# dayne-2stacks/Fingerprint-Matching-Code

Measured on AMD Instinct MI355X. Metric: graph-match pairs/sec @ n=256 kpts, batch=1024, 1 & 8 GPU, higher is better.
Workload: dtype bf16

## Files before the change

### fingerprint-matching-code_amd/_lib.py

```python
import ctypes
import os

_HERE = os.path.dirname(os.path.abspath(__file__))
LIB_PATH = os.environ.get("FPM_LIB_PATH") or os.path.join(_HERE, "libfpm_hip.so")

P = ctypes.c_void_p
I = ctypes.c_int
L = ctypes.c_long
F = ctypes.c_float

SIGNATURES = {
    "fpm_last_error": (ctypes.c_char_p, []),
    "fpm_version": (I, []),
    "fpm_device_sync": (I, []),
    "fpm_sinkhorn_log_fwd": (I, [P, L, L, L, P, L, L, L, P, P, I, I, I, I, F, I, P]),
    "fpm_sinkhorn_ws_bytes": (L, [I, I, I]),
    "fpm_sinkhorn_log_fwd_ws": (I, [P, L, L, L, P, L, L, L, P, P, I, I, I, I, F, I, P, L, P]),
    "fpm_soft_topk_fwd": (I, [P, L, L, P, P, P, I, I, I, I, F, P, L, L, P, P, L, L, P]),
    "fpm_topk_select": (I, [P, L, L, P, L, P, I, I, I, P, L, L, P, L, L, P]),
    "fpm_greedy_perm": (I, [P, L, I, P, I, I, I, P, L, L, P]),
    "fpm_gemm": (I, [I, P, L, L, P, P, L, L, I, I, I, I, I, P, P, P, L, L, P, P, P]),
    "fpm_cast_bf16": (I, [P, P, L, P]),
    "fpm_global_weights": (I, [P, L, P, L, I, I, I, P, L, P]),
    "fpm_coef_tanh": (I, [P, L, P, P, I, I, I, P, L, P]),
# ... 44 lines not shown
    "fpm_match_cls_train_bwd": (I, [P, P, I, I, I] + [P] * 21 + [P]),
    "fpm_gemm_norm_max": (I, [P, L, P, L, I, I, I, P, P, L, P, P, ctypes.c_float, I, P, P]),
    "fpm_gemm_norm_out": (I, [P, L, P, L, I, I, I, P, P, P, ctypes.c_float, I, P, L, P, L, P]),
    "fpm_affinity_ws_floats": (L, [I, I, I]),
    "fpm_perm_loss_fwd": (I, [P, L, L, P, L, L, P, P, I, I, I, P, P, P, P]),
    "fpm_perm_loss_bwd": (I, [P, L, L, P, L, L, P, P, I, I, I, P, P, P, P]),
    "fpm_affinity_fwd": (I, [P, L, P, L, P, I, P, P, I, I, I, I, P, P, I, P, L, P, L, P]),
    "fpm_gemm_x3out": (I, [P, L, P, L, I, I, I, I, P, P, P, ctypes.c_float, I, P, L, P, L, I, P]),
    "fpm_lsa_batch_host": (I, [P, L, L, P, P, I, I, P, I]),
    "fpm_lsa_submit": (L, [P, L, L, P, P, I, I, P, I]),
    "fpm_lsa_wait": (I, [L, I, ctypes.POINTER(ctypes.c_double)]),
    "fpm_lsa_batch_device": (I, [P, L, L, P, P, I, I, I, P, P, P]),
    "fpm_csr_dot_csc_to_dense": (I, [I, P, P, P, P, P, P, L, L, L, P, P]),
    "fpm_dense_dot_csc_to_dense": (I, [I, P, P, P, P, L, L, L, L, P, P]),
    "fpm_csr_dot_diag_to_csr": (I, [I, P, P, P, P, L, L, L, P, P]),
    "fpm_bilinear_diag": (I, [I, P, P, P, P, L, P, P, P, L, L, P, P]),
    "fpm_csr_dot_csc_to_csr_host": (L, [I, P, P, P, P, P, P, L, L, L, P, L, P, P]),
    "fpm_csr_dot_diag_to_csr_host": (I, [I, P, P, P, P, L, L, L, P]),
    "fpm_bilinear_diag_host": (I, [I, P, P, P, P, L, P, P, P, L, L, P]),
    "fpm_gconv_ws_floats": (L, [I, I, I]),
    "fpm_gconv_fwd": (I, [P, P, I, I, I, I, P, P, I, P, P, P]),
    "fpm_graph_words": (I, [I]),
    "fpm_graph_build": (I, [P, P, I, I, I, ctypes.c_double, P, P, P, P, P]),
    "fpm_graph_edges": (I, [P, P, P, P, I, I, ctypes.c_double, P, P, P, P, P, P, I, P]),
    "fpm_kron_pattern": (I, [P, P, L, P, P, L, I, I, I, I, P, P, P]),
    "fpm_feature_align_ws_floats": (L, [P, P]),
    "fpm_feature_align_fwd": (I, [P, P, P, P, P, P, P, P, I, F, F, P, P, L, P, P]),
    "fpm_feature_align_bwd": (I, [P, P, P, P, P, P, P, P, I, F, F, P, P, L, P, P, P, P, P, P]),
    "fpm_sinkhorn_bwd_ws_floats": (L, [I, I, I, I]),
    "fpm_sinkhorn_log_bwd": (I, [P, L, L, L, P, L, L, L, P, P, P, I, I, I, I, F, I, P, L, P]),
    "fpm_soft_topk_bwd_ws_floats": (L, [I, I, I]),
    "fpm_soft_topk_bwd": (I, [P, L, L, P, P, P, P, I, I, I, F, P, L, L, P, P, L, P, P]),
    "fpm_spline_plan_rows": (I, [P, L, L, ctypes.POINTER(P), ctypes.POINTER(P)]),
    "fpm_spline_conv_bwd_data": (I, [I, P, L, L, I, P, P, P, I, P, P, P, P, P, P, I, P]),
    "fpm_gather_transpose": (I, [I, P, L, P, L, I, P, L, P]),
    "fpm_spline_weight_pack": (I, [P, P, I, I, I, I, I, P, P]),
    "fpm_spline_conv_bwd_data_scatter": (I, [I, P, P, P, L, L, I, P, P, P, I, P, P, P, P, P, P, I, P]),
    "fpm_kron_agg": (I, [P, I, I, I, I, P, P, P, P, P, P, P, P, I, P, P]),
    "fpm_kron_gnn_layer_bwd_point": (I, [P, I, I, I, I, P, P, P, P, P, P, P]),
    "fpm_kron_gnn_layer_fwd_f64": (I, [P, I, I, I, I, I, P, P, P, P, P, P, P, P, P, P]),
    "fpm_sinkhorn_log_fwd_f64": (I, [P, I, L, L, L, P, L, L, L, P, L, L, L, P, P, I, I, I, I, ctypes.c_double, I, P]),
    "fpm_node_classifier_f64": (I, [P, I, I, I, P, P, P, P, P]),
    "fpm_crossset_attn_row_f64": (I, [P, L, L, I, I, I, P, P, I, P, P, P, P, P, P]),
    "fpm_gemm_f64": (I, [P, I, P, I, P, P, I, I, I, I, I, P]),
    "fpm_instnorm_f64": (I, [P, P, I, I, I, P, P, P, P, ctypes.c_double, P, P, P]),
    "fpm_afau_head_f64": (I, [P, P, P, I, I, P, P, P, P, P, P, P, P, P, P]),
    "fpm_soft_topk_fwd_f64": (I, [P, L, L, P, P, P, I, I, I, I, ctypes.c_double, P, L, P, L, L, P, P, L, L, P]),
    "fpm_profile_enable": (I, [I]),
    "fpm_profile_enabled": (I, []),
    "fpm_profile_read": (I, [ctypes.POINTER(ctypes.c_double), ctypes.POINTER(ctypes.c_double),
                             ctypes.POINTER(I)]),
}

for _op, _probe in (("score", [P, I]), ("pairs", [P, P, P, I])):
    for _kernel, _ws in (("", []), ("_wide", [P, L]), ("_stream", [P, L])):
        for _rows in ("", "_rows16"):
            SIGNATURES["fpm_coarse_%s%s%s" % (_op, _kernel, _rows)] = (
                I, [P, P, P, I, I] + _probe + [P, I, F, P] + _ws + [P])

_lib = None


class FpmError(RuntimeError):
    pass


# ... 24 lines not shown
```

### fingerprint-matching-code_amd/csrc/gemm.hip

```cpp
#include "gemm_phase.h"
#include <cstdlib>
#include <cstring>

namespace fpm {
int& gemm_bn256_min();
}
int& gemm_store_sc1_flag();

extern "C" int fpm_gemm(int dtype, const void* A, long lda, long sA, const int* a_rows, const void* B, long ldb,
                        long sB, int M, int N, int K, int batch, int epi, const float* bias, float* Cf, void* Ct,
                        long ldc, long sC, const int* n1, const int* n2, void* stream) {
    using namespace fpm;
    FPM_CHECK_ARG(dtype == 0 || dtype == 1, "gemm: dtype must be 0 (f32) or 1 (bf16)");
    FPM_CHECK_ARG(M >= 0 && N > 0 && K > 0 && batch >= 0, "gemm: bad sizes M=%d N=%d K=%d", M, N, K);
    FPM_CHECK_ARG(K % (dtype ? 8 : 4) == 0, "gemm: K=%d must be a multiple of %d", K, dtype ? 8 : 4);
    FPM_CHECK_ARG(lda % (dtype ? 8 : 4) == 0 && ldb % (dtype ? 8 : 4) == 0, "gemm: lda/ldb must keep rows 16-B aligned");
    FPM_CHECK_ARG((epi != EPI_AFFINITY && epi != EPI_HALF_AFFINITY) || (n1 && n2),
                  "gemm: affinity epilogues need n1/n2");
    FPM_CHECK_ARG(epi >= EPI_STORE && epi <= EPI_HALF_AFFINITY, "gemm: bad epilogue %d", epi);
    if (M == 0 || batch == 0) return 0;
    GemmParams p = {};
    p.A = A; p.lda = lda; p.sA = sA; p.a_rows = a_rows;
    p.B = B; p.ldb = ldb; p.sB = sB; p.sB_seg = 0;
    p.row_scale = nullptr;
// ... 24 lines not shown
            else if (f32) FPM_BIG(256, EPI_STORE, true);
            else {
                const int S = phase ? gemm_walk_strip(p) : 0;
                p.store_sc1 = gemm_store_sc1_flag();
                if (S != 0) gemm_walk_launch(p, S, batch, st);
                else FPM_BIG(256, EPI_STORE, false);
            }
        } else {
            if (epi == EPI_RELU) { if (f32) FPM_BIG(128, EPI_RELU, true); else FPM_BIG(128, EPI_RELU, false); }
            else { if (f32) FPM_BIG(128, EPI_STORE, true); else FPM_BIG(128, EPI_STORE, false); }
        }
#undef FPM_BIG
        return check_launch("fpm_gemm");
    }
    p.remap_mtiles = (M + GBM - 1) / GBM;
    dim3 grid(remap_grid(N, p.remap_mtiles), 1, batch);
    if (dtype == 0) hipLaunchKernelGGL((gemm_kernel<float, false>), grid, dim3(GTHREADS), 0, st, p);
    else hipLaunchKernelGGL((gemm_kernel<bf16_t, false>), grid, dim3(GTHREADS), 0, st, p);
    return check_launch("fpm_gemm");
}

namespace fpm {
int& gemm_phase_flag() {
    static int on = [] {
        const char* e = getenv("FPM_GEMM_PHASE");
        return e ? atoi(e) : 1;
    }();
    return on;
}

int& gemm_walk_flag() {
    static int v = [] {
        const char* e = getenv("FPM_GEMM_WALK");
        return e ? atoi(e) : GW_AUTO;
    }();
    return v;
}

int gemm_cu_count() {
    static int cus = [] {
        int dev = 0, n = 0;
        if (hipGetDevice(&dev) != hipSuccess ||
            hipDeviceGetAttribute(&n, hipDeviceAttributeMultiprocessorCount, dev) != hipSuccess || n <= 0)
            n = 256;
        return n;
    }();
    return cus;
}

int& gemm_bn256_min() {
    static int v = [] {
        const char* e = getenv("FPM_GEMM_BN256_MIN");
        return e ? atoi(e) : 512;
    }();
    return v;
}
}

extern "C" int fpm_gemm_norm_max(const void* A, long lda, const void* B, long ldb, int M, int N, int K,
                                 const float* bias, const float* res, long ldres, const float* nw, const float* nb,
                                 float eps, int P, float* gmax, void* stream) {
    using namespace fpm;
    FPM_CHECK_ARG(P == G2_BM || 2 * P == G2_BM, "gemm_norm_max: P=%d must be %d or %d (one or two pairs per tile)", P,
                  G2_BM, G2_BM / 2);
    FPM_CHECK_ARG(M >= 0 && M % P == 0 && N > 0 && K > 0 && K % G2_BK == 0, "gemm_norm_max: bad sizes M=%d N=%d K=%d",
                  M, N, K);
    FPM_CHECK_ARG(lda % 8 == 0 && ldb % 8 == 0 && ldres >= N, "gemm_norm_max: bad strides");
// ... 126 lines not shown
    else if (key && !strcmp(key, "combine_npb")) f = &combine_npb_flag();
    else if (key && !strcmp(key, "sinkhorn_bwd_reg")) f = &sinkhorn_bwd_reg_flag();
    else if (key && !strcmp(key, "sinkhorn_fast")) f = &sinkhorn_fast_flag();
    else if (key && !strcmp(key, "sinkhorn_lform")) f = &sinkhorn_lform_flag();
    else if (key && !strcmp(key, "topk_fast")) f = &soft_topk_fast_flag();
    else if (key && !strcmp(key, "afau_attn_v")) f = &afau_attn_v_flag();
    else if (key && !strcmp(key, "gnn_store_sc1")) f = &gnn_store_sc1_flag();
    else if (key && !strcmp(key, "combine_store_sc1")) f = &combine_store_sc1_flag();
    else if (key && !strcmp(key, "gemm_store_sc1")) f = &gemm_store_sc1_flag();
    else if (key && !strcmp(key, "combine_lds_kb")) f = &combine_lds_kb_flag();
    else if (key && !strcmp(key, "gnn_mlp_off")) f = &gnn_mlp_off_flag();
    else if (key && !strcmp(key, "outer_sum_vec")) f = &outer_sum_vec_flag();
    else if (key && !strcmp(key, "gnn_sweeps")) f = &gnn_sweeps_flag();
    else if (key && !strcmp(key, "scatter_f32_rows")) f = &scatter_f32_rows_flag();
    else if (key && !strcmp(key, "scatter_batch")) f = &scatter_batch_flag();
    else if (key && !strcmp(key, "afau_head_split")) f = &afau_head_split_flag();
    if (!f) {
        fpm::set_error("fpm_set_tuning: unknown key '%s'", key ? key : "(null)");
        return -1;
    }
    if (f == &gnn_mlp_off_flag() && value != 0) {
        const char* e = getenv("FPM_TIMING_PROBES");
        if (!e || strcmp(e, "1") != 0) {
            fpm::set_error("fpm_set_tuning: '%s' is a timing probe with wrong results; set FPM_TIMING_PROBES=1 "
                           "to allow it", key);
            return -1;
        }
    }
    const int prev = *f;
    *f = value;
    return prev;
}

namespace {
__global__ void cast_bf16_kernel(const float* __restrict__ x, bf16_t* __restrict__ y, long n) {
    long i = (long)blockIdx.x * blockDim.x + threadIdx.x;
    long stride = (long)gridDim.x * blockDim.x;
    for (; i < n; i += stride) y[i] = fpm::f2bf(x[i]);
}

__global__ __launch_bounds__(256) void cast_bf16_v8_kernel(const float4* __restrict__ x, uint4* __restrict__ y, long n8) {
    const long i = (long)blockIdx.x * blockDim.x + threadIdx.x;
    if (i >= n8) return;
    const float4 a = x[2 * i], b = x[2 * i + 1];
    uint4 o;
    o.x = (uint32_t)fpm::f2bf(a.x) | ((uint32_t)fpm::f2bf(a.y) << 16);
    o.y = (uint32_t)fpm::f2bf(a.z) | ((uint32_t)fpm::f2bf(a.w) << 16);
    o.z = (uint32_t)fpm::f2bf(b.x) | ((uint32_t)fpm::f2bf(b.y) << 16);
    o.w = (uint32_t)fpm::f2bf(b.z) | ((uint32_t)fpm::f2bf(b.w) << 16);
    y[i] = o;
}
}

extern "C" int fpm_cast_bf16(const float* x, void* y, long n, void* stream) {
    if (n <= 0) return 0;
    if (n % 8 == 0 && ((uintptr_t)x & 15) == 0 && ((uintptr_t)y & 15) == 0) {
        const long n8 = n / 8;
        hipLaunchKernelGGL(cast_bf16_v8_kernel, dim3((unsigned)((n8 + 255) / 256)), dim3(256), 0, (hipStream_t)stream,
                           (const float4*)x, (uint4*)y, n8);
        return fpm::check_launch("fpm_cast_bf16");
    }
    long blocks = (n + 255) / 256;
    if (blocks > 65536) blocks = 65536;
    hipLaunchKernelGGL(cast_bf16_kernel, dim3(blocks), dim3(256), 0, (hipStream_t)stream, x, (bf16_t*)y, n);
    return fpm::check_launch("fpm_cast_bf16");
}
// ... 122 lines not shown
```

### fingerprint-matching-code_amd/csrc/gemm_core.h

```cpp
#pragma once
#include "fpm_common.h"

namespace fpm {

enum GemmEpi : int {
    EPI_STORE = 0,
    EPI_RELU = 1,
    EPI_TANH = 2,
    EPI_AFFINITY = 3,
    EPI_HALF_AFFINITY = 4,
    EPI_NORM_MAX = 5,
    EPI_NORM_OUT = 6,
};

struct GemmParams {
    const void* A;
    long lda, sA;
    const int* a_rows;
    const void* B;
    long ldb, sB, sB_seg;
    const float* row_scale;
    int M, N, K, nseg;
    const int* tile_info;
    const int* group_off;
    int epi;
    const float* bias;
    float* Cf;
    void* Ct;
    long ldc, sC;
    const int* n1;
    const int* n2;
    int remap_mtiles;
    const float* res;
    const float* nw;
    const float* nb;
    float eps;
    float* gmax;
    long ldt;
    int split;
    int norm_p;
    int store_sc1;
    int remap_cm;
    int walk;
    const int* tile_count;
    int walk_cus;
};

constexpr int REMAP_MIN = 32;
inline unsigned remap_grid(int N, int mtiles) {
    long nt = (N + 127) / 128, chunk = 4 * nt;
    long t = nt * mtiles;
    if (mtiles < REMAP_MIN) return (unsigned)t;
    return (unsigned)((t + 8 * chunk - 1) / (8 * chunk) * (8 * chunk));
}
__device__ __forceinline__ int remap_tile(int nt, int mtiles, int cm = 4) {
    if (mtiles < REMAP_MIN) return blockIdx.x;
    const int chunk = cm * nt;
    const int i = blockIdx.x >> 3;
    return ((i / chunk) * 8 + (blockIdx.x & 7)) * chunk + (i % chunk);
}

typedef __bf16 bf16x8_t __attribute__((ext_vector_type(8)));
typedef float f32x4_t __attribute__((ext_vector_type(4)));

template <typename T> struct TileCfg;
template <> struct TileCfg<float> {
    static constexpr int BK = 32;
    static constexpr int EPC = 4;
};
template <> struct TileCfg<bf16_t> {
    static constexpr int BK = 64;
    static constexpr int EPC = 8;
};

constexpr int GBM = 128, GBN = 128, GTHREADS = 256;
constexpr int LDS_ROW_BYTES = 144;
constexpr int LDS_TILE_BYTES = GBM * LDS_ROW_BYTES;

// ... 197 lines not shown
```

### fingerprint-matching-code_amd/csrc/gemm_phase.h

```cpp
#pragma once
#include <type_traits>
#include "gemm_big.h"

namespace fpm {

constexpr int GP_HALF = 128 * 128;
constexpr int GP_SMEM = g2_max(8 * GP_HALF, G2_BM * (2 * 256 + 16));
constexpr int GP_MIN_KTILES = 2;

#define FPM_VMCNT(N) asm volatile("s_waitcnt vmcnt(" #N ")" ::: "memory")

#ifdef GP_PROBE
__device__ unsigned long long* gp_probe_buf;
#define GP_STAMP(k)                                                                                   \
    do {                                                                                              \
        const unsigned long long t_ = __builtin_amdgcn_s_memtime();                                   \
        if (threadIdx.x == 0 && gp_probe_buf)                                                         \
            gp_probe_buf[((long)blockIdx.z * gridDim.x + blockIdx.x) * 8 + (k)] = t_;                   \
    } while (0)
#else
#define GP_STAMP(k)
#endif

#ifndef GP_STAGGER
// ... 271 lines not shown
                            *(float*)(smem + r * ROW + c * 4) =
                                g2_epi<EPI, HB>(p.bias, acc[h][g][fm][fn][j], row0 + h * 128 + r, n, n1b, n2b);
                        }
                    }
        };
#pragma unroll
        for (int h = 0; h < 2; ++h) {
            if (p.bias) image(h, std::true_type{});
            else image(h, std::false_type{});
            __syncthreads();
#pragma unroll 4
            for (int it = 0; it < 128 * CH / G2_THREADS; ++it) {
                const int idx = it * G2_THREADS + tid;
                const int r = idx / CH, ch = idx % CH;
                const int gr = row0 + h * 128 + r;
                if (gr < row_end && n0 + ch * 4 < p.N) {
                    uint4 v = *(const uint4*)(smem + r * ROW + ch * 16);
                    *(uint4*)(Cf + (long)gr * p.ldc + n0 + ch * 4) = v;
                }
            }
            __syncthreads();
        }
    }
}

constexpr int GW_SMEM = 8 * GP_HALF;
constexpr int GW_MAX_S = 2;

__host__ __device__ inline int gemm_walk_rule(int tiles, int wgs, int cus) {
    const long r1 = ((long)tiles * wgs + cus - 1) / cus, r2 = ((long)((tiles + 1) / 2) * wgs + cus - 1) / cus;
    return 2 * r2 * 7 <= r1 * 8 ? 2 : 1;
}

#ifdef GP_PROBE
#define GW_STAMP(k) do { if (ti == 0) GP_STAMP(k); } while (0)
#else
#define GW_STAMP(k)
#endif

template <bool SC1>
__global__ __launch_bounds__(G2_THREADS, 1) void gemm_walk_kernel(GemmParams p) {
    constexpr int BN = 256;
    __shared__ __attribute__((aligned(16))) unsigned char smem[GW_SMEM];
    const int tid = threadIdx.x, lane = tid & 63, wave = tid >> 6;
    const int wr = wave >> 2, wc = wave & 3;
    const int batch = blockIdx.z;

    const int nt = p.N / BN;
    int mtiles = p.remap_mtiles;
    if (p.tile_count) mtiles = *p.tile_count < mtiles ? *p.tile_count : mtiles;
    const int S = p.walk > 0 ? p.walk : gemm_walk_rule(mtiles, nt * (int)gridDim.z, p.walk_cus);
    const int strips = (mtiles + S - 1) / S;
    const int i = blockIdx.x >> 3;
    const int strip = (i / nt) * 8 + (blockIdx.x & 7), ntile = i % nt;
    if (strip >= strips) return;
    int t_row0[GW_MAX_S], t_rend[GW_MAX_S], t_grp[GW_MAX_S];
    unsigned ok = 0;
#pragma unroll
    for (int j = 0; j < GW_MAX_S; ++j) {
        const int mt = strip * S + j;
        t_row0[j] = 0; t_rend[j] = 0; t_grp[j] = 0;
        if (j < S && mt < mtiles) {
            if (p.tile_info) {
                const int g = p.tile_info[2 * mt];
                if (g >= 0) {
                    t_grp[j] = g;
                    t_row0[j] = p.tile_info[2 * mt + 1];
                    t_rend[j] = p.group_off[g + 1];
                    ok |= 1u << j;
                }
            } else {
                t_row0[j] = mt * G2_BM;
                t_rend[j] = p.M;
                ok |= 1u << j;
            }
        }
    }
    if (!ok) return;
    constexpr int m_end = GW_MAX_S;
    auto next_valid = [&](int j) __attribute__((always_inline)) {
        const unsigned r = j < GW_MAX_S ? ok >> j : 0u;
        return r ? j + __builtin_ctz(r) : GW_MAX_S;
    };
    auto pick = [&](const int (&t)[GW_MAX_S], int j) __attribute__((always_inline)) {
        return j == 0 ? t[0] : t[1];
    };
    int m = next_valid(0);

    const int n0 = ntile * BN;
    const bf16_t* A = (const bf16_t*)p.A + (long)batch * p.sA;
    const unsigned char* Bb = (const unsigned char*)((const bf16_t*)p.B + (long)batch * p.sB);
    bf16_t* Ct = (bf16_t*)p.Ct + (long)batch * p.sC;

// ... 203 lines not shown
    for (;;) {
        const bool has_next = mn < m_end;
        GW_STAMP(0);
        if (GP_STAGGER && wr == 1) __builtin_amdgcn_s_barrier();
        int k1 = G2_BK;
        for (int t = 0; t < T - 2; ++t, ++u, k1 += G2_BK) ktile(u, k1, 6, 6, 6, 6, CUR, CUR);
        ktile(u, k1, 6, 6, 6, has_next ? 6 : 4, CUR, has_next ? NEXT : NONE);
        GW_STAMP(1);
        ktile(u + 1, 0, has_next ? 6 : 2, has_next ? 6 : 0, -1, -1, has_next ? NEXT : NONE, NONE);
        ++u;
        if (GP_STAGGER && wr == 0) __builtin_amdgcn_s_barrier();
        GW_STAMP(2);
        if (p.bias) epilogue(u & 1, std::true_type{});
        else epilogue(u & 1, std::false_type{});
        GW_STAMP(3);
        if (!has_next) break;
        m = mn; mn = m_end;
        row0 = row0n; row_end = row_endn; bg = bgn;
#pragma unroll
        for (int h = 0; h < 2; ++h)
#pragma unroll
            for (int i = 0; i < 2; ++i) ar[h][i] = arn[h][i];
        issue(0, u & 1, ar, bg, G2_BK);
        issue(2, u & 1, ar, bg, G2_BK);
        FPM_VMCNT(4);
        zero_acc();
        __builtin_amdgcn_s_barrier();
        GW_STAMP(4);
        ++u;
#ifdef GP_PROBE
        ++ti;
#endif
    }
}

#undef FPM_VMCNT

int& gemm_phase_flag();
inline bool use_gemm_phase(int K) { return gemm_phase_flag() != 0 && K / G2_BK >= GP_MIN_KTILES; }

constexpr int GW_AUTO = 8;
int& gemm_walk_flag();
int gemm_cu_count();
inline int gemm_walk_strip(const GemmParams& p) {
    const int f = gemm_walk_flag();
    if (f <= 1 || !use_gemm_phase(p.K) || p.N % 256 != 0 || !p.Ct || p.Cf || p.epi != EPI_STORE) return 0;
    if ((long)p.N * p.ldb * 2 >= (1L << 31) || (long)G2_BM * p.ldc * 2 >= (1L << 31) || p.lda >= (1L << 31)) return 0;
    return f < GW_AUTO ? 2 : GW_AUTO;
}
inline void gemm_walk_launch(GemmParams p, int S, int batch, hipStream_t st) {
    const long nt = p.N / 256;
    p.walk_cus = gemm_cu_count();
    p.walk = S == 2 || p.remap_mtiles * nt * batch >= 8L * gemm_cu_count() ? 2 : 0;
    const int strips = p.walk ? (p.remap_mtiles + 1) / 2 : p.remap_mtiles;
    const dim3 grid((unsigned)((strips + 7) / 8 * 8 * nt), 1, batch);
    if (p.store_sc1) hipLaunchKernelGGL((gemm_walk_kernel<true>), grid, dim3(G2_THREADS), 0, st, p);
    else hipLaunchKernelGGL((gemm_walk_kernel<false>), grid, dim3(G2_THREADS), 0, st, p);
}

}
```

### fingerprint-matching-code_amd/csrc/spline.hip

```cpp
#include "gemm_phase.h"

#include <vector>

namespace {

struct ProfRec {
    hipEvent_t a, b;
    int slot;
};
bool g_prof_on = false;
std::vector<ProfRec> g_prof;
int* g_prof_rows = nullptr;
constexpr int PROF_MAX = 4096;

constexpr int NCELL = 26;

struct PlanLayout {
    long mask, indeg, dslot, basis_e, grp_e, blk_cnt, cell_off, rowid, arows, tile_info, tile_info2, dst_ptr, csr_e,
        nbr_local, rows4, basis4, total;
    long nblk, max_rows, max_tiles, max_tiles2;
};

__host__ __device__ inline long al(long x) { return (x + 255) & ~255L; }

// ... 1372 lines not shown
extern "C" int fpm_profile_enabled(void) { return g_prof_on ? 1 : 0; }

extern "C" int fpm_profile_read(double* ms_total, double* flops_total, int* count) {
    double ms = 0.0, fl = 0.0;
    for (auto& r : g_prof) {
        float t = 0.f;
        if (hipEventSynchronize(r.b) != hipSuccess || hipEventElapsedTime(&t, r.a, r.b) != hipSuccess) {
            fpm::set_error("fpm_profile_read: event query failed");
            return 2;
        }
        int rows = 0;
        if (hipMemcpy(&rows, g_prof_rows + r.slot, sizeof(int), hipMemcpyDeviceToHost) != hipSuccess) {
            fpm::set_error("fpm_profile_read: row count read failed");
            return 2;
        }
        ms += t;
        fl += 2.0 * rows * 768.0 * 768.0;
        (void)hipEventDestroy(r.a);
        (void)hipEventDestroy(r.b);
    }
    if (count) *count = (int)g_prof.size();
    g_prof.clear();
    if (ms_total) *ms_total = ms;
    if (flops_total) *flops_total = fl;
    return 0;
}

extern "C" int fpm_cast_bf16(const float* x, void* out, long n, void* stream);

extern "C" int fpm_spline_plan_rows(void* ws, long E, long num_nodes, int** arows, int** cell_off) {
    PlanLayout L = plan_layout(E, num_nodes);
    *arows = (int*)((char*)ws + L.arows);
    *cell_off = (int*)((char*)ws + L.cell_off);
    return 0;
}

extern "C" int fpm_spline_plan_edges(void* ws, long E, long num_nodes, int** csr_e, int** rows4, float** basis4) {
    PlanLayout L = plan_layout(E, num_nodes);
    *csr_e = (int*)((char*)ws + L.csr_e);
    *rows4 = (int*)((char*)ws + L.rows4);
    *basis4 = (float*)((char*)ws + L.basis4);
    return 0;
}

extern "C" int fpm_spline_conv_bwd_data_scatter(int dtype, const void* plan_ws, const void* rplan_ws,
                                                const int* argmax, long E, long num_nodes, int nmax,
                                                const int* nvalid, const void* Wb, const void* y_ws, int mode,
                                                const float* gout, const float* hout, float* dY, void* dY_op,
                                                float* dXrows, float* dX, int accumulate, void* stream);

extern "C" int fpm_spline_conv_bwd_data(int dtype, const void* plan_ws, long E, long num_nodes, int nmax,
                                        const int* nvalid, const void* Wb, const void* y_ws, int mode,
                                        const float* gout, const float* hout, float* dY, void* dY_op,
                                        float* dXrows, float* dX, int accumulate, void* stream) {
    return fpm_spline_conv_bwd_data_scatter(dtype, plan_ws, nullptr, nullptr, E, num_nodes, nmax, nvalid, Wb, y_ws,
                                            mode, gout, hout, dY, dY_op, dXrows, dX, accumulate, stream);
}

int& scatter_f32_rows_flag() {
    static int v = [] {
        const char* e = getenv("FPM_SCATTER_F32_ROWS");
        return e ? atoi(e) : 0;
    }();
    return v;
}

// ... 126 lines not shown
```

### fingerprint-matching-code_amd/ops.py

```python
import ctypes

import torch

from . import _lib

F32, BF16 = 0, 1
EPI_STORE, EPI_RELU, EPI_TANH, EPI_AFFINITY, EPI_HALF_AFFINITY = 0, 1, 2, 3, 4
EPI_NORM_OUT = 6


def _p(t):
    return ctypes.c_void_p(0 if t is None else t.data_ptr())


def _stream(t=None):
    dev = t.device if t is not None else torch.device("cuda")
    return ctypes.c_void_p(torch.cuda.current_stream(dev).cuda_stream)


def _dev(*ts):
    for t in ts:
        if t is not None and not t.is_cuda:
            raise _lib.FpmError("fpm op called with a CPU tensor: the HIP path has no CPU fallback")

# ... 1089 lines not shown
              dp.stride(1), dp.stride(2), _p(ds), _p(n1), _p(n2), B, n1max, n2max, int(iters), float(tau),
              int(bool(dummy_row)), _p(ws), ws.numel(), _stream(s))
    return ds


def soft_topk_bwd(ss, n1, n2, k, steps, tau, dds):
    _dev(ss, n1, n2, k, steps, dds)
    B, n1max, n2max = ss.shape
    if ss.stride(2) != 1 or dds.stride(2) != 1 or tuple(dds.shape) != (B, n1max, n2max):
        raise _lib.FpmError("soft_topk_bwd: (B, n1max, n2max) views with unit column stride expected")
    lib = _lib.load()
    ws = torch.empty(max(int(lib.fpm_soft_topk_bwd_ws_floats(B, n1max, n2max)), 1), device=ss.device,
                     dtype=torch.float32)
    status = torch.zeros(B, device=ss.device, dtype=torch.int32)
    dss = torch.empty(B, n1max, n2max, device=ss.device, dtype=torch.float32)
    _lib.call("fpm_soft_topk_bwd", _p(ss), ss.stride(0), ss.stride(1), _p(n1), _p(n2), _p(k), _p(steps), B, n1max,
              n2max, float(tau), _p(dds), dds.stride(0), dds.stride(1), _p(dss), _p(ws), ws.numel(), _p(status),
              _stream(ss))
    if int(status.sum()):
        raise _lib.FpmError("soft_topk_bwd: forward ran more steps than the backward replay holds")
    return dss


def spline_plan_rows(plan, E, num_nodes):
    a, c = ctypes.c_void_p(), ctypes.c_void_p()
    _lib.call("fpm_spline_plan_rows", _p(plan), E, num_nodes, ctypes.byref(a), ctypes.byref(c))
    base = plan.data_ptr()
    oa, oc = a.value - base, c.value - base
    arows = plan[oa:].view(torch.int32)
    cell_off = plan[oc:oc + 4 * 27].view(torch.int32)
    return arows, cell_off


def spline_plan_edges(plan, E, num_nodes):
    a, r, b = ctypes.c_void_p(), ctypes.c_void_p(), ctypes.c_void_p()
    _lib.call("fpm_spline_plan_edges", _p(plan), E, num_nodes, ctypes.byref(a), ctypes.byref(r), ctypes.byref(b))
    base = plan.data_ptr()
    oa, orr, ob = a.value - base, r.value - base, b.value - base
    csr_e = plan[oa:oa + 4 * E].view(torch.int32)
    rows4 = plan[orr:orr + 16 * E].view(torch.int32).view(E, 4)
    basis4 = plan[ob:ob + 16 * E].view(torch.float32).view(E, 4)
    return csr_e, rows4, basis4


def spline_conv_bwd_data(x_op, plan, E, num_nodes, nmax, nvalid, Wb, y_ws, mode, gout, hout, dY, dY_op, dXrows, dX,
                         accumulate=False, rplan=None, argmax=None):
    _dev(plan, nvalid, Wb, y_ws, gout, dY, dXrows, dX)
    code = _code(x_op)
    if _code(Wb) != code or tuple(Wb.shape) != (26, 768, 768):
        raise _lib.FpmError("spline_conv_bwd: Wb must be (26, 768, 768) in the operand dtype")
    if mode == 0 and hout is None:
        raise _lib.FpmError("spline_conv_bwd: mode 0 needs the layer output")
    if (rplan is None) != (argmax is None):
        raise _lib.FpmError("spline_conv_bwd: rplan and argmax go together")
    _lib.call("fpm_spline_conv_bwd_data_scatter", code, _p(plan), _p(rplan), _p(argmax), E, num_nodes, nmax,
              _p(nvalid), _p(Wb), _p(y_ws), int(mode), _p(gout), _p(hout), _p(dY), _p(dY_op), _p(dXrows), _p(dX),
              int(bool(accumulate)), _stream(gout))


def kron_agg(X, C, B, n1max, n2max, tcsr1, tcsr2, q1, q2, n1, n2, adjoint, out, accumulate=False):
    _dev(X, n1, n2, out)
    _lib.call("fpm_kron_agg", _p(X), int(C), int(B), int(n1max), int(n2max), ctypes.c_void_p(tcsr1[0]),
              ctypes.c_void_p(tcsr1[1]), ctypes.c_void_p(tcsr2[0]), ctypes.c_void_p(tcsr2[1]), ctypes.c_void_p(q1),
              ctypes.c_void_p(q2), _p(n1), _p(n2), int(bool(adjoint)) | (2 if accumulate else 0), _p(out), _stream(X))
    return out

# ... 104 lines not shown
```

### include/fpm.h

```cpp
#ifndef FPM_H_
#define FPM_H_

#ifdef __cplusplus
extern "C" {
#endif

const char* fpm_last_error(void);
int fpm_version(void);
int fpm_device_sync(void);

int fpm_sinkhorn_log_fwd(const float* s, long s_sb, long s_si, long s_sj, float* out, long o_sb, long o_si,
                         long o_sj, const int* n1, const int* n2, int B, int n1max, int n2max, int iters,
                         float tau, int dummy_row, void* stream);
long fpm_sinkhorn_ws_bytes(int B, int n1max, int n2max);
int fpm_sinkhorn_log_fwd_ws(const float* s, long s_sb, long s_si, long s_sj, float* out, long o_sb, long o_si,
                            long o_sj, const int* n1, const int* n2, int B, int n1max, int n2max, int iters,
                            float tau, int dummy_row, void* ws, long ws_bytes, void* stream);

int fpm_soft_topk_fwd(const float* ss, long s_sb, long s_ld, const int* n1, const int* n2, const float* k, int B,
                      int n1max, int n2max, int iters, float tau, float* out, long o_sb, long o_ld, int* steps_out,
                      float* out2, long o2_sb, long o2_ld, void* stream);

int fpm_topk_select(const float* ds, long d_sb, long d_ld, const int* assign, long a_sb, const float* k, int B,
                    int n1max, int n2max, float* perm, long p_sb, long p_ld, float* lsa_out, long l_sb, long l_ld,
// ... 226 lines not shown
                     float* score, void* stream);
int fpm_coarse_pairs_wide(const float* y, const long* row_off, const int* idx, int G, int B, const float* yq,
                          const long* qrow_off, const int* qidx, int Q, const float* coef, int iters, float tau,
                          float* score, void* ws, long ws_bytes, void* stream);
int fpm_coarse_pairs_stream(const float* y, const long* row_off, const int* idx, int G, int B, const float* yq,
                            const long* qrow_off, const int* qidx, int Q, const float* coef, int iters, float tau,
                            float* score, void* ws, long ws_bytes, void* stream);
int fpm_coarse_pairs_rows16(const void* y16, const long* row_off, const int* idx, int G, int B, const float* yq,
                            const long* qrow_off, const int* qidx, int Q, const float* coef, int iters, float tau,
                            float* score, void* stream);
int fpm_coarse_pairs_wide_rows16(const void* y16, const long* row_off, const int* idx, int G, int B, const float* yq,
                                 const long* qrow_off, const int* qidx, int Q, const float* coef, int iters,
                                 float tau, float* score, void* ws, long ws_bytes, void* stream);
int fpm_coarse_pairs_stream_rows16(const void* y16, const long* row_off, const int* idx, int G, int B,
                                   const float* yq, const long* qrow_off, const int* qidx, int Q, const float* coef,
                                   int iters, float tau, float* score, void* ws, long ws_bytes, void* stream);

int fpm_profile_enable(int on);
int fpm_profile_enabled(void);
int fpm_profile_read(double* ms_total, double* flops_total, int* count);

int fpm_lsa_batch_device(const float* s, long sb, long ld, const int* n1, const int* n2, int B, int n1max, int n2max,
                         int* assign, int* status, void* stream);

long fpm_sinkhorn_bwd_ws_floats(int B, int n1max, int n2max, int iters);
int fpm_sinkhorn_log_bwd(const float* s, long s_sb, long s_si, long s_sj, const float* dp, long d_sb, long d_si,
                         long d_sj, float* ds, const int* n1, const int* n2, int B, int n1max, int n2max, int iters,
                         float tau, int dummy_row, float* ws, long ws_floats, void* stream);
long fpm_soft_topk_bwd_ws_floats(int B, int n1max, int n2max);
int fpm_soft_topk_bwd(const float* ss, long sb, long ld, const int* n1, const int* n2, const float* k,
                      const int* steps, int B, int n1max, int n2max, float tau, const float* dds, long db, long dld,
                      float* dss, float* ws, long ws_floats, int* status, void* stream);
int fpm_spline_plan_rows(void* plan_ws, long E, long num_nodes, int** arows, int** cell_off);
int fpm_spline_conv_bwd_data(int dtype, const void* plan_ws, long E, long num_nodes, int nmax, const int* nvalid,
                             const void* Wb, const void* y_ws, int mode, const float* gout, const float* hout,
                             float* dY, void* dY_op, float* dXrows, float* dX, int accumulate, void* stream);
int fpm_spline_conv_bwd_data_scatter(int dtype, const void* plan_ws, const void* rplan_ws, const int* argmax, long E,
                                     long num_nodes, int nmax, const int* nvalid, const void* Wb, const void* y_ws,
                                     int mode, const float* gout, const float* hout, float* dY, void* dY_op,
                                     float* dXrows, float* dX, int accumulate, void* stream);
int fpm_gather_transpose(int dtype, const void* in, long ldi, const int* rows, long Q, int C, void* out, long ldo,
                         void* stream);
int fpm_spline_weight_pack(const float* weight, const float* root, int K, int Cin, int Cout, int transpose, int dtype,
                           void* out, void* stream);
int fpm_kron_agg(const float* X, int C, int B, int n1max, int n2max, const int* tptr1, const int* tnbr1,
                 const int* tptr2, const int* tnbr2, const int* q1, const int* q2, const int* n1, const int* n2,
                 int adjoint, float* out, void* stream);

int fpm_kron_gnn_layer_bwd_point(const float* X, int C, int B, int n1max, int n2max, const float* dXn, const float* dz,
                                 const float* params, float* dX, float* dagg, float* V, void* stream);

int fpm_lsa_batch_host(const float* s, long sb, long ld, const int* n1, const int* n2, int B, int n1max, int* assign,
                       int nthreads);
long fpm_lsa_submit(const float* s, long sb, long ld, const int* n1, const int* n2, int B, int n1max, int* assign,
                    int nthreads);
int fpm_lsa_wait(long ticket, int block, double* seconds);

#ifdef __cplusplus
}
#endif
#endif
```

Baseline: 32030.

## Add mixed paired/single tile walk schedule and default GEMM walk to uniform

Extends the GEMM walk kernel so that workgroups can process a mix of paired and single M-tiles, using an XCD-aware cost model to choose a split that balances work across CUs. The default walk mode changes from auto to a new uniform mode, which keeps plain pairing without mixing. It also adds host-side helpers that expose the schedule and spline tile tables for inspection. The new per-block plan computation adds some index arithmetic at kernel entry, and changing the default alters which tile grouping production GEMMs use.

```diff
diff --git a/fingerprint-matching-code_amd/_lib.py b/fingerprint-matching-code_amd/_lib.py
--- a/fingerprint-matching-code_amd/_lib.py
+++ b/fingerprint-matching-code_amd/_lib.py
@@ -100,6 +100,8 @@
     "fpm_soft_topk_bwd_ws_floats": (L, [I, I, I]),
     "fpm_soft_topk_bwd": (I, [P, L, L, P, P, P, P, I, I, I, F, P, L, L, P, P, L, P, P]),
     "fpm_spline_plan_rows": (I, [P, L, L, ctypes.POINTER(P), ctypes.POINTER(P)]),
+    "fpm_spline_plan_tiles": (I, [P, L, L, ctypes.POINTER(P), ctypes.POINTER(P), ctypes.POINTER(L)]),
+    "fpm_gemm_walk_schedule": (I, [I, I, I, I, I, I, P, P]),
     "fpm_spline_conv_bwd_data": (I, [I, P, L, L, I, P, P, P, I, P, P, P, P, P, P, I, P]),
     "fpm_gather_transpose": (I, [I, P, L, P, L, I, P, L, P]),
     "fpm_spline_weight_pack": (I, [P, P, I, I, I, I, I, P, P]),
diff --git a/fingerprint-matching-code_amd/csrc/gemm.hip b/fingerprint-matching-code_amd/csrc/gemm.hip
--- a/fingerprint-matching-code_amd/csrc/gemm.hip
+++ b/fingerprint-matching-code_amd/csrc/gemm.hip
@@ -80,7 +80,7 @@
 int& gemm_walk_flag() {
     static int v = [] {
         const char* e = getenv("FPM_GEMM_WALK");
-        return e ? atoi(e) : GW_AUTO;
+        return e ? atoi(e) : GW_UNIFORM;
     }();
     return v;
 }
@@ -273,6 +273,30 @@
     return prev;
 }
 
+extern "C" int fpm_gemm_walk_schedule(int mode, int tiles, int table_tiles, int nt, int batch, int cus, int* counts,
+                                      int* out) {
+    using namespace fpm;
+    FPM_CHECK_ARG(mode >= 2 && tiles >= 0 && table_tiles >= tiles && nt > 0 && batch > 0 && cus > 0 && out,
+                  "gemm_walk_schedule: bad arguments");
+    const int m = mode < GW_AUTO ? 2 : mode == GW_MIXED || mode == GW_UNIFORM ? mode : GW_AUTO;
+    const GemmWalkConfig c = gemm_walk_config(m, table_tiles, nt, batch, cus);
+    const GemmWalkPlan pl = gemm_walk_plan(tiles, nt * batch, cus, c.walk, c.mix);
+    const int grid_units = (c.units + 7) / 8 * 8;
+    out[0] = c.walk; out[1] = c.mix; out[2] = grid_units;
+    out[3] = pl.paired; out[4] = pl.units; out[5] = pl.cost; out[6] = pl.mixed;
+    out[7] = gemm_walk_rule(tiles, nt * batch, cus);
+    if (counts) {
+        for (int t = 0; t < tiles; ++t) counts[t] = 0;
+        for (int u = 0; u < grid_units; ++u) {
+            int first = 0, len = 0;
+            if (!gemm_walk_tiles(u, tiles, nt * batch, cus, c.walk, c.mix, first, len)) continue;
+            for (int j = 0; j < len; ++j)
+                if (first + j < tiles) ++counts[first + j];
+        }
+    }
+    return 0;
+}
+
 namespace {
 __global__ void cast_bf16_kernel(const float* __restrict__ x, bf16_t* __restrict__ y, long n) {
     long i = (long)blockIdx.x * blockDim.x + threadIdx.x;
diff --git a/fingerprint-matching-code_amd/csrc/gemm_core.h b/fingerprint-matching-code_amd/csrc/gemm_core.h
--- a/fingerprint-matching-code_amd/csrc/gemm_core.h
+++ b/fingerprint-matching-code_amd/csrc/gemm_core.h
@@ -44,6 +44,7 @@
     int walk;
     const int* tile_count;
     int walk_cus;
+    int walk_mix;
 };
 
 constexpr int REMAP_MIN = 32;
diff --git a/fingerprint-matching-code_amd/csrc/gemm_phase.h b/fingerprint-matching-code_amd/csrc/gemm_phase.h
--- a/fingerprint-matching-code_amd/csrc/gemm_phase.h
+++ b/fingerprint-matching-code_amd/csrc/gemm_phase.h
@@ -327,6 +327,76 @@
     return 2 * r2 * 7 <= r1 * 8 ? 2 : 1;
 }
 
+constexpr int GW_XCDS = 8;
+constexpr int GW_MIX_OFF = 0, GW_MIX_MODEL = 1, GW_MIX_FORCE = 2;
+struct GemmWalkPlan {
+    int paired;
+    int units;
+    int cost;
+    int mixed;
+};
+__host__ __device__ inline GemmWalkPlan gemm_walk_plan(int tiles, int wgs, int cus, int fallback, int mix) {
+    const unsigned T = (unsigned)tiles, w = (unsigned)wgs, c = (unsigned)cus;
+    const unsigned r1 = (T * w + c - 1) / c, r2 = ((T + 1) / 2 * w + c - 1) / c;
+    const int c1 = (int)(8 * r1), c2 = (int)(14 * r2);
+    const int S = fallback ? fallback : (c2 <= c1 ? 2 : 1);
+    GemmWalkPlan pl;
+    pl.mixed = 0;
+    pl.paired = S == 2 ? tiles : 0;
+    pl.units = S == 2 ? (tiles + 1) / 2 : tiles;
+    pl.cost = S == 2 ? c2 : c1;
+    const unsigned cx = c / GW_XCDS;
+    if (mix == GW_MIX_OFF || cx == 0) return pl;
+    const unsigned a = T / 2 / GW_XCDS;
+    const unsigned R = a * w / cx;
+    const unsigned p8 = R * cx / w;
+    const unsigned P = 2 * GW_XCDS * p8, n = T - P;
+    if (mix == GW_MIX_FORCE) {
+        pl.mixed = p8 > 0 && n > 0;
+        pl.paired = (int)P;
+        pl.units = (int)(P / 2 + n);
+        pl.cost = p8 == 0 ? c1 : n == 0 ? c2 : 0;
+    }
+    if (p8 == 0 || n == 0) return pl;
+    const unsigned n1 = (n + GW_XCDS - 1) / GW_XCDS;
+    const unsigned q = (p8 + n1) * w;
+    const int cm = (int)(14 * R + 8 * (q > R * cx ? (q - R * cx + cx - 1) / cx : 0));
+    if (mix == GW_MIX_FORCE) { pl.cost = cm; return pl; }
+    if (cm < c1 && cm < c2) {
+        pl.mixed = 1;
+        pl.paired = (int)P;
+        pl.units = (int)(P / 2 + n);
+        pl.cost = cm;
+    }
+    return pl;
+}
+__host__ __device__ inline void gemm_walk_unit(const GemmWalkPlan& pl, int unit, int& first, int& len) {
+    const int np = (pl.paired + 1) / 2;
+    first = unit < np ? 2 * unit : pl.paired + (unit - np);
+    len = unit < np ? 2 : 1;
+}
+__host__ __device__ inline int gemm_walk_slack(int wgs, int cus) {
+    const int cx = cus / GW_XCDS;
+    return 17 + 16 * ((cx + wgs - 1) / wgs);
+}
+__host__ __device__ inline bool gemm_walk_tiles(int unit, int mtiles, int wgs, int cus, int walk, int mix, int& first,
+                                                int& len) {
+    if (unit >= mtiles) return false;
+    if (walk == 2 && mix == GW_MIX_OFF) {
+        first = 2 * unit;
+        len = 2;
+        return first < mtiles;
+    }
+    if (mix != GW_MIX_FORCE) {
+        const bool pairs = walk == 2 || (walk == 0 && gemm_walk_plan(mtiles, wgs, cus, 0, GW_MIX_OFF).paired != 0);
+        if (pairs && 2 * unit >= mtiles + gemm_walk_slack(wgs, cus)) return false;
+    }
+    const GemmWalkPlan pl = gemm_walk_plan(mtiles, wgs, cus, walk, mix);
+    if (unit >= pl.units) return false;
+    gemm_walk_unit(pl, unit, first, len);
+    return true;
+}
+
 #ifdef GP_PROBE
 #define GW_STAMP(k) do { if (ti == 0) GP_STAMP(k); } while (0)
 #else
@@ -344,16 +414,16 @@
     const int nt = p.N / BN;
     int mtiles = p.remap_mtiles;
     if (p.tile_count) mtiles = *p.tile_count < mtiles ? *p.tile_count : mtiles;
-    const int S = p.walk > 0 ? p.walk : gemm_walk_rule(mtiles, nt * (int)gridDim.z, p.walk_cus);
-    const int strips = (mtiles + S - 1) / S;
     const int i = blockIdx.x >> 3;
-    const int strip = (i / nt) * 8 + (blockIdx.x & 7), ntile = i % nt;
-    if (strip >= strips) return;
+    const int unit = (i / nt) * 8 + (blockIdx.x & 7), ntile = i % nt;
+    int strip0, S;
+    if (!gemm_walk_tiles(unit, mtiles, nt * (int)gridDim.z, p.walk_cus, p.walk, p.walk_mix, strip0, S)) return;
+    GP_STAMP(5);
     int t_row0[GW_MAX_S], t_rend[GW_MAX_S], t_grp[GW_MAX_S];
     unsigned ok = 0;
 #pragma unroll
     for (int j = 0; j < GW_MAX_S; ++j) {
-        const int mt = strip * S + j;
+        const int mt = strip0 + j;
         t_row0[j] = 0; t_rend[j] = 0; t_grp[j] = 0;
         if (j < S && mt < mtiles) {
             if (p.tile_info) {
@@ -623,6 +693,7 @@
         ++ti;
 #endif
     }
+    GP_STAMP(6);
 }
 
 #undef FPM_VMCNT
@@ -630,20 +701,37 @@
 int& gemm_phase_flag();
 inline bool use_gemm_phase(int K) { return gemm_phase_flag() != 0 && K / G2_BK >= GP_MIN_KTILES; }
 
-constexpr int GW_AUTO = 8;
+constexpr int GW_AUTO = 8, GW_MIXED = 9, GW_UNIFORM = 10;
 int& gemm_walk_flag();
 int gemm_cu_count();
 inline int gemm_walk_strip(const GemmParams& p) {
     const int f = gemm_walk_flag();
     if (f <= 1 || !use_gemm_phase(p.K) || p.N % 256 != 0 || !p.Ct || p.Cf || p.epi != EPI_STORE) return 0;
     if ((long)p.N * p.ldb * 2 >= (1L << 31) || (long)G2_BM * p.ldc * 2 >= (1L << 31) || p.lda >= (1L << 31)) return 0;
-    return f < GW_AUTO ? 2 : GW_AUTO;
-}
-inline void gemm_walk_launch(GemmParams p, int S, int batch, hipStream_t st) {
+    return f < GW_AUTO ? 2 : f == GW_MIXED || f == GW_UNIFORM ? f : GW_AUTO;
+}
+struct GemmWalkConfig {
+    int walk, mix, units;
+};
+inline GemmWalkConfig gemm_walk_config(int mode, int table_tiles, long nt, int batch, int cus) {
+    GemmWalkConfig c;
+    c.walk = mode == 2 || table_tiles * nt * batch >= 8L * cus ? 2 : 0;
+    c.mix = mode == GW_MIXED ? GW_MIX_FORCE : mode == GW_AUTO ? GW_MIX_MODEL : GW_MIX_OFF;
+    if (mode == 2 || table_tiles * nt * batch >= (1L << 31)) c.mix = GW_MIX_OFF;
+    if (c.walk == 2 && c.mix == GW_MIX_OFF) c.units = (table_tiles + 1) / 2;
+    else if (c.walk == 2 && c.mix == GW_MIX_MODEL)
+        c.units = (int)((table_tiles + (long)gemm_walk_slack((int)(nt * batch), cus)) / 2 + 1);
+    else c.units = table_tiles;
+    if (c.units > table_tiles) c.units = table_tiles;
+    return c;
+}
+inline void gemm_walk_launch(GemmParams p, int mode, int batch, hipStream_t st) {
     const long nt = p.N / 256;
     p.walk_cus = gemm_cu_count();
-    p.walk = S == 2 || p.remap_mtiles * nt * batch >= 8L * gemm_cu_count() ? 2 : 0;
-    const int strips = p.walk ? (p.remap_mtiles + 1) / 2 : p.remap_mtiles;
+    const GemmWalkConfig c = gemm_walk_config(mode, p.remap_mtiles, nt, batch, p.walk_cus);
+    p.walk = c.walk;
+    p.walk_mix = c.mix;
+    const int strips = c.units;
     const dim3 grid((unsigned)((strips + 7) / 8 * 8 * nt), 1, batch);
     if (p.store_sc1) hipLaunchKernelGGL((gemm_walk_kernel<true>), grid, dim3(G2_THREADS), 0, st, p);
     else hipLaunchKernelGGL((gemm_walk_kernel<false>), grid, dim3(G2_THREADS), 0, st, p);
diff --git a/fingerprint-matching-code_amd/csrc/spline.hip b/fingerprint-matching-code_amd/csrc/spline.hip
--- a/fingerprint-matching-code_amd/csrc/spline.hip
+++ b/fingerprint-matching-code_amd/csrc/spline.hip
@@ -1428,6 +1428,15 @@
     PlanLayout L = plan_layout(E, num_nodes);
     *arows = (int*)((char*)ws + L.arows);
     *cell_off = (int*)((char*)ws + L.cell_off);
+    return 0;
+}
+
+extern "C" int fpm_spline_plan_tiles(void* ws, long E, long num_nodes, int** tile_info, int** tile_count,
+                                     long* max_tiles) {
+    PlanLayout L = plan_layout(E, num_nodes);
+    *tile_info = (int*)((char*)ws + L.tile_info2);
+    *tile_count = (int*)((char*)ws + L.cell_off) + NCELL + 2;
+    *max_tiles = L.max_tiles2;
     return 0;
 }
 
diff --git a/fingerprint-matching-code_amd/ops.py b/fingerprint-matching-code_amd/ops.py
--- a/fingerprint-matching-code_amd/ops.py
+++ b/fingerprint-matching-code_amd/ops.py
@@ -1145,6 +1145,27 @@
     return arows, cell_off
 
 
+def spline_plan_tiles(plan, E, num_nodes):
+    t, c, m = ctypes.c_void_p(), ctypes.c_void_p(), ctypes.c_long()
+    _lib.call("fpm_spline_plan_tiles", _p(plan), E, num_nodes, ctypes.byref(t), ctypes.byref(c), ctypes.byref(m))
+    base = plan.data_ptr()
+    ot, oc = t.value - base, c.value - base
+    tile_info = plan[ot:ot + 8 * m.value].view(torch.int32).view(m.value, 2)
+    tile_count = plan[oc:oc + 4].view(torch.int32)
+    return tile_info, tile_count
+
+
+def gemm_walk_schedule(mode, tiles, nt, batch, cus, table_tiles=None, counts=False):
+    out = (ctypes.c_int * 8)()
+    cnt = torch.zeros(max(tiles, 1), dtype=torch.int32) if counts else None
+    _lib.call("fpm_gemm_walk_schedule", int(mode), int(tiles), int(tiles if table_tiles is None else table_tiles),
+              int(nt), int(batch), int(cus), cnt.data_ptr() if counts else None, ctypes.cast(out, ctypes.c_void_p))
+    r = dict(zip(("walk", "mix", "grid_units", "paired", "units", "cost", "mixed", "rule"), list(out)))
+    if counts:
+        r["counts"] = cnt[:tiles]
+    return r
+
+
 def spline_plan_edges(plan, E, num_nodes):
     a, r, b = ctypes.c_void_p(), ctypes.c_void_p(), ctypes.c_void_p()
     _lib.call("fpm_spline_plan_edges", _p(plan), E, num_nodes, ctypes.byref(a), ctypes.byref(r), ctypes.byref(b))
diff --git a/include/fpm.h b/include/fpm.h
--- a/include/fpm.h
+++ b/include/fpm.h
@@ -282,6 +282,8 @@
                       const int* steps, int B, int n1max, int n2max, float tau, const float* dds, long db, long dld,
                       float* dss, float* ws, long ws_floats, int* status, void* stream);
 int fpm_spline_plan_rows(void* plan_ws, long E, long num_nodes, int** arows, int** cell_off);
+int fpm_spline_plan_tiles(void* plan_ws, long E, long num_nodes, int** tile_info, int** tile_count, long* max_tiles);
+int fpm_gemm_walk_schedule(int mode, int tiles, int table_tiles, int nt, int batch, int cus, int* counts, int* out);
 int fpm_spline_conv_bwd_data(int dtype, const void* plan_ws, long E, long num_nodes, int nmax, const int* nvalid,
                              const void* Wb, const void* y_ws, int mode, const float* gout, const float* hout,
                              float* dY, void* dY_op, float* dXrows, float* dX, int accumulate, void* stream);
```

Result: slower. 30370 (-5.2%).
